# szaguldo-kamaz/FRI-ReinforcementLearning-C

Hardware: AMD Instinct MI355X
Metric: rule-distance evals/sec (rules x envs) (higher is better)
Workload: dtype f64; 1 GPU; cfg4_acrobot_64k_x_8k_per_gpu; nant=5, universe_len=41, rules_per_env=65536, envs_per_gpu=8192, exact_hits=4, dist_backend=none, world_size=1

## Files before the change

fri-reinforcementlearning-c_amd/csrc/device_common.h:

```cpp
#pragma once

#include <hip/hip_runtime.h>
#include <stdint.h>

#include "../../include/frirl_hip.h"

#define FRIRL_WAVE 64
#define FRIRL_BLOCK 256
#define FRIRL_WAVES_PER_BLOCK (FRIRL_BLOCK / FRIRL_WAVE)

namespace frirl {

__device__ __forceinline__ unsigned snap_index(const double *__restrict__ uni, int len, double point, double div)
{
    const int low = (int)((point - uni[0]) / div);
    if (low < 0) return 0u;
    if (low >= len) return (unsigned)(len - 1);
    if (low + 1 >= len) return (unsigned)low;
    const double d1 = uni[low] - point;
    const double d2 = uni[low + 1] - point;
    return (fabs(d1) <= fabs(d2)) ? (unsigned)low : (unsigned)(low + 1);
}

__device__ __forceinline__ double universe_div(const double *__restrict__ uni, int U)
// ... 95 lines not shown
namespace frirl_host {
void set_error(const char *fmt, ...);
int check_device();
int check_launch(const char *what);
int check_tables(const frirl_hip_tables *t);
int check_rulebases(const frirl_hip_tables *t, const frirl_hip_rulebases *b);
int check_demo_kind(const frirl_hip_tables *t, const frirl_hip_agent *agent, const char *who);
int check_grid_len(const frirl_hip_tables *t, const frirl_hip_agent *agent, const char *who);
int check_policy_args(const frirl_hip_tables *t, const frirl_hip_rulebases *b, const frirl_hip_agent *agent, const char *who);
int check_policy_io(const frirl_hip_agent_io *io, bool begin, const char *who);
#define FRIRL_POLICY_NANT_CASES(M) M(2) M(3) M(4) M(5) M(6) M(7) M(8)
int check_agent_shape(const frirl_hip_tables *t, const frirl_hip_rulebases *b, const frirl_hip_agent *agent, const frirl_hip_envs *envs,
                      const char *who);
inline hipStream_t as_stream(void *s) { return reinterpret_cast<hipStream_t>(s); }

struct DeviceGuard {
    int prev = -1;
    DeviceGuard() { if (hipGetDevice(&prev) != hipSuccess) { prev = -1; (void)hipGetLastError(); } }
    ~DeviceGuard() { if (prev >= 0) (void)hipSetDevice(prev); }
    DeviceGuard(const DeviceGuard &) = delete;
    DeviceGuard &operator=(const DeviceGuard &) = delete;
};

struct Options {
    int no_uidx;
    int rd_unroll;
    int rd_chunk;
    int rd_nt;
    int rd_persist;
    int rd_order;
    int rd_packed;
    int rd_sqdiff;
    int rd_qpass;
    int rd_prepass;
    int rd_coded;
    int step_wave;
    int step_track;
    int lanes_slices;
    int lanes_wpe;
    int rollout_group;
    int rollout_slices;
    int rollout_resident;
    int rollout_cap;
    int rollout_pair;
    int rollout_wps;
    int rollout_batch_resident;
    int rollout_batch_resident_rules;
    int rollout_batch_slices;
    int rollout_record_slices;
    int policy_group;
    int policy_slices;
    int learn_slices;
    int learn_alone;
    int learn_persistent;
    int multi_loopback;
    int mirror_sync;
    int no_many;
};
const Options &opts();
}
```

fri-reinforcementlearning-c_amd/csrc/learn.hip:

```cpp
#include "learn_kernel.h"

using namespace frirl_host;
int frirl_check_episode(const frirl_hip_tables *t, const frirl_hip_rulebases *b, const frirl_hip_agent *agent, const frirl_hip_envs *envs, const char *who);

static long learn_lanes()
{
    int cus = 256;
    { int dev = 0, n = 0; if (hipGetDevice(&dev) == hipSuccess && hipDeviceGetAttribute(&n, hipDeviceAttributeMultiprocessorCount, dev) == hipSuccess && n > 0) cus = n; }
    return (long)cus * 4 * 2 * FRIRL_WAVE;
}

static int learn_slices(int nlive)
{
    { const int v = opts().learn_slices; if (v == 1 || v == 2 || v == 4 || v == 8 || v == 16 || v == 32 || v == 64) return v; }
    const long lanes = learn_lanes();
    int H = 1;
    while (H < 64 && (long)nlive * (2 * H) <= lanes) H *= 2;
    return H;
}

extern "C" int frirl_hip_learn_plan(int32_t nlive, int32_t mean_rules, int32_t *slices, int32_t *agents_per_launch)
{
    if (nlive < 1 || !slices || !agents_per_launch) { set_error("frirl_hip_learn_plan: bad arguments"); return FRIRL_HIP_EINVAL; }
    const long lanes = learn_lanes();
// ... 33 lines not shown
}

static size_t learn_entries(int nlive, int maxR, int H)
{
    const int EPW = FRIRL_WAVE / H;
    const size_t tiles = ((size_t)nlive + EPW - 1) / EPW, njmax = ((size_t)maxR + H - 1) / H;
    return tiles * (njmax + frirl::LR_PADROWS) * 64;
}

extern "C" size_t frirl_hip_learn_workspace_bytes(int32_t nant, int32_t E, int32_t maxR, int32_t A)
{
    if (nant < 1 || E < 1 || maxR < 1 || A < 1) return 0;
    size_t m = 0;
    for (int H : {1, 2, 4, 8, 16, 32, 64}) { const size_t n = learn_entries(E, maxR, H); m = n > m ? n : m; }
    return m * (16 + 8 + 8) + 256;
}

#ifdef LEARN_TIMING
static unsigned long long *learn_timing_buffer()
{
    static unsigned long long *p = nullptr;
    if (!p) { if (hipMalloc(&p, 16 * 8) != hipSuccess) return nullptr; (void)hipMemset(p, 0, 16 * 8); }
    return p;
}
extern "C" int frirl_hip_learn_timing(unsigned long long *out16)
{
    unsigned long long *p = learn_timing_buffer();
    if (!p || hipMemcpy(out16, p, 16 * 8, hipMemcpyDeviceToHost) != hipSuccess) return FRIRL_HIP_EINVAL;
    (void)hipMemset(p, 0, 16 * 8);
    return FRIRL_HIP_OK;
}
#endif

extern "C" int frirl_hip_learn_run(const frirl_hip_tables *t, const frirl_hip_rulebases *b, const frirl_hip_agent *agent, const frirl_hip_envs *envs,
                                   const frirl_hip_convergence *conv, const int32_t *live, int32_t nlive, int32_t budget_steps, int32_t max_episodes,
                                   int64_t *work, int64_t *steps_total, void *workspace, size_t workspace_bytes, void *stream)
{
    int rc = frirl_check_episode(t, b, agent, envs, "frirl_hip_learn_run");
    if (rc) return rc;
    if (!conv || !conv->prev_nrules || !conv->prev_steps || !conv->prev_reward || !conv->prev_rconc || !conv->converged || !conv->episodes) { set_error("frirl_hip_learn_run: NULL convergence state"); return FRIRL_HIP_EINVAL; }
    if (!frirl_hip_learn_supported(t->nant, t->U, agent->A, agent->p, agent->env_kind)) { set_error("frirl_hip_learn_run: shape nant=%d U=%d A=%d p=%d not covered (use frirl_hip_episode_run_lanes)", t->nant, t->U, agent->A, agent->p); return FRIRL_HIP_EINVAL; }
    if (!b->uidx) { set_error("frirl_hip_learn_run: needs the 16-bit index mirror (frirl_hip_rulebases.uidx)"); return FRIRL_HIP_EINVAL; }
    if (nlive < 1 || nlive > b->E || budget_steps < 0 || max_episodes < 1) { set_error("frirl_hip_learn_run: nlive=%d / budget=%d / max_episodes=%d", nlive, budget_steps, max_episodes); return FRIRL_HIP_EINVAL; }
    if (!workspace || (reinterpret_cast<uintptr_t>(workspace) & 15)) { set_error("frirl_hip_learn_run: workspace must be a 16-byte aligned device buffer"); return FRIRL_HIP_EINVAL; }
    const size_t need = frirl_hip_learn_workspace_bytes(t->nant, nlive, b->maxR, agent->A);
    if (workspace_bytes < need) { set_error("frirl_hip_learn_run: workspace %zu B < %zu B (frirl_hip_learn_workspace_bytes)", workspace_bytes, need); return FRIRL_HIP_EINVAL; }
    hipStream_t s = as_stream(stream);
    frirl::LearnArgs la = {};
    la.u = t->u; la.ve = t->ve; la.U = t->U;
    la.Ti = static_cast<uint32_t *>(workspace);
    la.live = live; la.nlive = nlive;
    la.rb = b->rb; la.uidx = b->uidx; la.nrules = b->nrules; la.maxR = b->maxR;
    la.work = work; la.steps_total = steps_total; la.budget = budget_steps; la.max_episodes = max_episodes;
#ifdef LEARN_TIMING
    la.timing = learn_timing_buffer();
#endif
    int H = learn_slices(nlive);
    if (H < learn_min_slices(agent->A)) H = learn_min_slices(agent->A);
    if (t->nant == 3) frirl_learn_launch_mountaincar(H, t, b, agent, envs, conv, la, s);
    else if (agent->A == 3) { if (H <= 8) frirl_learn_launch_acrobot_lo(H, t, b, agent, envs, conv, la, s); else frirl_learn_launch_acrobot_hi(H, t, b, agent, envs, conv, la, s); }
    else { if (H <= 8) frirl_learn_launch_cartpole_lo(H, t, b, agent, envs, conv, la, s); else frirl_learn_launch_cartpole_hi(H, t, b, agent, envs, conv, la, s); }
    return check_launch("frirl_hip_learn_run");
}


namespace {
constexpr int LQ_BLOCK = 1024, LQ_BINS = 4096;

__global__ void learn_queue_init_kernel(int32_t *q, int n)
{
    for (int i = blockIdx.x * blockDim.x + threadIdx.x; i < n; i += gridDim.x * blockDim.x) q[i] = i;
}

__global__ __launch_bounds__(LQ_BLOCK) void learn_queue_sort_kernel(const int32_t *__restrict__ q, int take, const int32_t *__restrict__ nrules, int shift,
                                                                    int32_t *__restrict__ live)
{
    __shared__ int bins[LQ_BINS];
    __shared__ int part[LQ_BLOCK];
    for (int i = threadIdx.x; i < LQ_BINS; i += LQ_BLOCK) bins[i] = 0;
    __syncthreads();
    auto key = [&](int e) { const int k = nrules[e] >> shift; return k < 0 ? 0 : (k >= LQ_BINS ? LQ_BINS - 1 : k); };
    for (int i = threadIdx.x; i < take; i += LQ_BLOCK) atomicAdd(&bins[key(q[i])], 1);
    __syncthreads();
    constexpr int PER = LQ_BINS / LQ_BLOCK;
    int loc[PER], sum = 0;
#pragma unroll
    for (int x = 0; x < PER; x++) { loc[x] = sum; sum += bins[threadIdx.x * PER + x]; }
    part[threadIdx.x] = sum;
    __syncthreads();
    for (int off = 1; off < LQ_BLOCK; off <<= 1) {
        const int v = threadIdx.x >= off ? part[threadIdx.x - off] : 0;
        __syncthreads();
        part[threadIdx.x] += v;
        __syncthreads();
    }
    const int base = part[threadIdx.x] - sum;
#pragma unroll
    for (int x = 0; x < PER; x++) bins[threadIdx.x * PER + x] = base + loc[x];
    __syncthreads();
    for (int i = threadIdx.x; i < take; i += LQ_BLOCK) { const int e = q[i]; live[atomicAdd(&bins[key(e)], 1)] = e; }
}

__global__ __launch_bounds__(LQ_BLOCK) void learn_queue_next_kernel(const int32_t *__restrict__ q, int n, int take, const int32_t *__restrict__ live,
                                                                    const int32_t *__restrict__ converged, const int32_t *__restrict__ episodes, int max_episodes,
                                                                    const int32_t *__restrict__ nrules, const int32_t *__restrict__ status, uint8_t *refused,
                                                                    int32_t *__restrict__ nq, long long *counters)
// ... 85 lines not shown
```

fri-reinforcementlearning-c_amd/csrc/learn_kernel.h:

```cpp
#pragma once
#include "sweeps.h"
#include "envs.h"
#include <type_traits>

namespace frirl {

#ifndef LEARN_UR
#define LEARN_UR 2
#endif
constexpr int LR_BLOCK = 256;
constexpr int LR_PADROWS = 16;
constexpr int LR_WPB = LR_BLOCK / FRIRL_WAVE;
constexpr int LR_MW = 16;

struct LearnArgs {
    const double *u, *ve;
    int U;
    uint32_t *Ti;
    double *Tq;
    double *Tp;
    const int32_t *live;
    int nlive, tiles, njmax;
    double *rb;
    uint16_t *uidx;
    int32_t *nrules;
    int maxR;
    int64_t *work;
    int64_t *steps_total;
    int budget;
    long long *sum_rules;
    int max_episodes;
#ifdef LEARN_TIMING
    unsigned long long *timing;
#endif
};
#ifdef LEARN_TIMING
#define LT_MARK(i) do { const unsigned long long now_ = clock64(); if ((__ffsll((long long)__ballot(1)) - 1) == lane) { tim_s[wave][i] += now_ - tim_s[wave][15]; tim_s[wave][15] = now_; } } while (0)
#else
#define LT_MARK(i) do { } while (0)
#endif

template <int NANT, int BITS>
__global__ __launch_bounds__(256) void learn_import_kernel(const LearnArgs la, int H, const double *__restrict__ prev_rconc)
{
    constexpr int FPW = Packed<BITS>::FPW, W = Packed<BITS>::words(NANT);
    const int tile = blockIdx.x, EPW = FRIRL_WAVE / H;
    const int lane = threadIdx.x & 63, il = lane / H, h = lane % H;
    const int slot = tile * EPW + il;
    const bool exists = slot < la.nlive;
    const int e = exists ? (la.live ? la.live[slot] : slot) : 0;
    const int R = exists ? la.nrules[e] : 0;
    const int nj = (R + H - 1) / H;
    if (threadIdx.x < 64 && h == 0 && exists) atomicAdd(reinterpret_cast<unsigned long long *>(la.sum_rules), (unsigned long long)R);
    int njw = nj;
    for (int off = 32; off > 0; off >>= 1) { const int o = __shfl_xor(njw, off, FRIRL_WAVE); njw = o > njw ? o : njw; }
    for (int j = threadIdx.x / 64; j < njw; j += 4) {
        const int r = j * H + h;
        uint32_t w[W];
#pragma unroll
        for (int x = 0; x < W; x++) w[x] = 0u;
        double q = 0.0, p = 0.0;
        if (r < R) {
#pragma unroll
            for (int k = 0; k < NANT; k++) w[k / FPW] |= (uint32_t)la.uidx[((size_t)e * NANT + k) * la.maxR + r] << (BITS * (k % FPW));
            q = la.rb[((size_t)e * (NANT + 1) + NANT) * la.maxR + r];
            p = prev_rconc[(size_t)e * la.maxR + r];
        }
        const size_t o = ((size_t)tile * (la.njmax + LR_PADROWS) + LR_PADROWS + j) * 64 + lane;
#pragma unroll
        for (int x = 0; x < W; x++) la.Ti[o * W + x] = w[x];
        la.Tq[o] = q;
        la.Tp[o] = p;
    }
}

template <int NANT>
__global__ __launch_bounds__(256) void learn_export_kernel(const LearnArgs la, int H, double *__restrict__ prev_rconc)
{
    constexpr int nant = NANT;
    const int tile = blockIdx.x, EPW = FRIRL_WAVE / H;
    const int lane = threadIdx.x & 63, il = lane / H, h = lane % H;
    const int slot = tile * EPW + il;
    const bool exists = slot < la.nlive;
    const int e = exists ? (la.live ? la.live[slot] : slot) : 0;
    const int R = exists ? la.nrules[e] : 0;
    const int nj = (R + H - 1) / H;
    int njw = nj;
    for (int off = 32; off > 0; off >>= 1) { const int o = __shfl_xor(njw, off, FRIRL_WAVE); njw = o > njw ? o : njw; }
    for (int j = threadIdx.x / 64; j < njw; j += 4) {
        const int r = j * H + h;
        if (r < R) {
            const size_t o = ((size_t)tile * (la.njmax + LR_PADROWS) + LR_PADROWS + j) * 64 + lane;
            la.rb[((size_t)e * (nant + 1) + nant) * la.maxR + r] = la.Tq[o];
            prev_rconc[(size_t)e * la.maxR + r] = la.Tp[o];
        }
    }
}

template <int NANT, int NA, int KIND, int H, int BITS, int WPS>
__global__ __launch_bounds__(LR_BLOCK, WPS) void learn_kernel(const LearnArgs la, const frirl_hip_agent ag, const frirl_hip_envs ev,
                                                              const frirl_hip_convergence cv)
{
    constexpr int NS = NANT - 1, EPW = FRIRL_WAVE / H;
    constexpr int FPW = Packed<BITS>::FPW, W = Packed<BITS>::words(NANT);
    constexpr int UR = LEARN_UR;
    using RecI = typename std::conditional<W == 1, uint32_t, typename std::conditional<W == 2, uint2, uint4>::type>::type;
    static_assert(BITS == 6 || BITS == 10, "the LDS tables are laid out for 6-bit (<= 64 points) or 10-bit (<= 1024 points: cartpole) universe indices");
    constexpr int TS = 1 << BITS;
    constexpr int MW = BITS == 6 ? LR_MW : LR_MW / 2;
    constexpr bool LU = KIND != FRIRL_HIP_ENV_CARTPOLE;
    constexpr int NCOLD = 2 * NS + 2 * NANT + 3 + 4;
    __shared__ double tab_s[(LU ? 2 : 1) * NANT * TS];
    __shared__ double grid_s[NANT * FRIRL_HIP_MAX_GRID];
    __shared__ double udiv[8];
    __shared__ unsigned aidx_s[NA];
    extern __shared__ __attribute__((aligned(16))) double cold_s[];
    __shared__ uint32_t mask_s[MW * LR_BLOCK];
    static_assert(32 % (2 * UR) == 0, "a flag word is filled by whole loop iterations");
    const int U = la.U, maxR = la.maxR;
    const int lane = threadIdx.x & (FRIRL_WAVE - 1), wave = threadIdx.x / FRIRL_WAVE;
    const int il = lane / H, h = lane % H;
    const int tile = blockIdx.x * LR_WPB + wave;
    const int slot = tile * EPW + il;
    const bool exists = tile < la.tiles && slot < la.nlive;
    const int e = exists ? (la.live ? la.live[slot] : slot) : 0;
    for (int i = threadIdx.x; i < NANT * U; i += LR_BLOCK) tab_s[(i / U) * TS + i % U] = la.ve[i];
    if (LU) for (int i = threadIdx.x; i < NANT * U; i += LR_BLOCK) tab_s[NANT * TS + (i / U) * TS + i % U] = la.u[i];
    for (int i = threadIdx.x; i < NANT * FRIRL_HIP_MAX_GRID; i += LR_BLOCK) grid_s[i] = ag.grid_values[i];
    __syncthreads();
    const double *ves = tab_s, *us;
    if constexpr (LU) us = tab_s + NANT * TS; else us = la.u;
    const int USTR = LU ? TS : U;
    if ((int)threadIdx.x < NANT) udiv[threadIdx.x] = universe_div(us + (size_t)threadIdx.x * USTR, U);
    __syncthreads();
    auto locate = [&](int k, double x, unsigned &idx) { const double *uni = us + (size_t)k * USTR; idx = snap_index(uni, U, x, udiv[k]); return ves[(size_t)k * TS + idx]; };
    if ((int)threadIdx.x < NA) aidx_s[threadIdx.x] = snap_index(us + (size_t)NS * USTR, U, grid_s[NS * FRIRL_HIP_MAX_GRID + threadIdx.x], udiv[NS]);
    __syncthreads();
    auto pack = [&](uint32_t (&w)[W], int k, unsigned idx) { w[k / FPW] |= (idx & ((1u << BITS) - 1u)) << (BITS * (k % FPW)); };
    const size_t tbase = ((size_t)(tile < la.tiles ? tile : 0) * (la.njmax + LR_PADROWS) + LR_PADROWS) * 64;
    const RecI *Ti_l = reinterpret_cast<const RecI *>(la.Ti) + tbase + lane;
    double *Tq_l = la.Tq + tbase + lane, *Tp_l = la.Tp + tbase + lane;
    RecI *Ti_g = reinterpret_cast<RecI *>(la.Ti) + tbase + il * H;
    double *Tq_g = la.Tq + tbase + il * H;
    const auto pk = pin_pow(PowC<NANT>());

    auto decode = [&](const RecI &x, double (&c)[NANT]) {
        uint32_t w[W];
        if constexpr (W == 1) { w[0] = x; } else if constexpr (W == 2) { w[0] = x.x; w[1] = x.y; } else { w[0] = x.x; w[1] = x.y; w[2] = x.z; if constexpr (W > 3) w[3] = x.w; }
#pragma unroll
        for (int k = 0; k < NANT; k++) {
            constexpr uint32_t FM = ((1u << BITS) - 1u) << 3;
            const int sh = BITS * (k % FPW);
            const uint32_t off = (sh >= 3 ? (w[k / FPW] >> (sh - 3)) : (w[k / FPW] << (3 - sh))) & FM;
            c[k] = *reinterpret_cast<const double *>(reinterpret_cast<const char *>(ves + k * TS) + off);
        }
    };
    auto fetch = [&](RecI(&xi)[UR], double(&xq)[UR], int jtop, bool needq) {
        const RecI *pi = Ti_l + (long)jtop * 64;
        const double *pq = Tq_l + (long)jtop * 64;
#pragma unroll
        for (int t = 0; t < UR; t++) {
            xi[t] = pi[-t * 64];
            xq[t] = needq ? pq[-t * 64] : 0.0;
        }
    };
    struct Pref { RecI i[UR]; double q[UR]; int jt; };
    auto slice_prefetch = [&](int R, bool needq) {
        Pref p;
        p.jt = (R - h + H - 1) / H - 1;
        if (p.jt < -1) p.jt = -1;
// ... 4 lines not shown
        constexpr bool FL = decltype(flags)::value;
        RecI ib[UR];
        double qb[UR];
        uint32_t cmask = 0u;
        auto consume = [&](const RecI(&xi)[UR], const double(&xq)[UR], int jtop) {
#pragma unroll
            for (int t = 0; t < UR; t++) {
                const int j = jtop - t;
                if constexpr (FL) {
                    uint32_t hi = 0u;
                    if (j >= 0) { double c[NANT]; decode(xi[t], c); hi = f(j * H + h, c, xq[t]); }
                    cmask = __builtin_amdgcn_alignbit(cmask, hi, 31);
                } else {
                    if (j >= 0) { double c[NANT]; decode(xi[t], c); f(j * H + h, c, xq[t]); }
                }
            }
        };
        int jt = p.jt;
        const int jt0 = jt, jtm = jt & 31;
        while (jt >= 0) {
            fetch(ib, qb, jt - UR, needq);
            consume(p.i, p.q, jt);
            fetch(p.i, p.q, jt - 2 * UR, needq);
            consume(ib, qb, jt - UR);
            jt -= 2 * UR;
            if constexpr (FL) {
                if ((jt & 31) == jtm) {
                    const int wd = ((jt0 - jt) >> 5) - 1;
                    if (wd < MW) mask_s[wd * LR_BLOCK + threadIdx.x] = cmask;
                }
            }
        }
        if constexpr (FL) {
            const int done = jt0 - jt, rem = done & 31;
            if (jt0 >= 0 && rem != 0 && (done >> 5) < MW) mask_s[(done >> 5) * LR_BLOCK + threadIdx.x] = cmask << (32 - rem);
        }
    };
    auto for_slice = [&](int R, bool needq, auto &&f) {
        Pref p = slice_prefetch(R, needq);
        for_slice_from(p, needq, f, std::false_type());
    };
    auto group_or = [&](bool v) -> bool {
        const unsigned long long b = __ballot(v ? 1 : 0);
        if constexpr (H == 64) return b != 0ull;
        else return ((b >> (il * H)) & ((1ull << H) - 1ull)) != 0ull;
    };

    double states[NS], q_ant[NANT], total = 0.0, prev_reward = 0.0;
    int R = 0, fus = 0, steps = 0, prevR = 0, prev_steps = 0, nep = 0, lsteps = 0;
    bool active = false, begin = false, converged = false, refused = false;
    uint32_t episode = 0;
    long long wmain = 0, wextra = 0;
    double thr = 0.0;
    constexpr long long STEP_RULES = 24 * H;
    const long long work_budget = (long long)la.budget * (*la.sum_rules / (la.nlive > 0 ? la.nlive : 1) + STEP_RULES);
    double ve1[NANT];
    uint32_t pk1[W];
    bool ongrid = false;
#pragma unroll
    for (int k = 0; k < NS; k++) states[k] = exists ? ev.states[(size_t)e * NS + k] : 0.0;
#pragma unroll
    for (int k = 0; k < NANT; k++) q_ant[k] = exists ? ev.q_ant[(size_t)e * NANT + k] : 0.0;
#pragma unroll
    for (int x = 0; x < W; x++) pk1[x] = 0u;
#pragma unroll
    for (int k = 0; k < NANT; k++) { unsigned i1; ve1[k] = locate(k, q_ant[k], i1); pack(pk1, k, i1); }
    if (exists) {
        R = la.nrules[e]; fus = ev.fus[e]; steps = ev.ep_steps[e]; total = ev.ep_reward[e];
        begin = ev.done[e] != 0;
        episode = ev.episode ? (uint32_t)ev.episode[e] : 0u;
        prevR = cv.prev_nrules[e]; prev_steps = cv.prev_steps[e]; prev_reward = cv.prev_reward[e];
        converged = cv.converged[e] != 0; nep = cv.episodes[e];
        active = !converged && nep < la.max_episodes - 1 && la.budget > 0;
    }

#ifdef LEARN_TIMING
    __shared__ unsigned long long tim_s[LR_WPB][16];
    if (lane < 16) tim_s[wave][lane] = 0ull;
    if (lane == 0) tim_s[wave][15] = clock64();
#endif
    while (__any(active ? 1 : 0)) {
        double cur[NS], cur_q[NANT], ve2[NS], reward = 0.0;
        uint32_t pk2[W];
        int success = 0;
#pragma unroll
        for (int x = 0; x < W; x++) pk2[x] = 0u;
        Pref pmain = slice_prefetch(active ? R : 0, true);
        if (active) {
            if (begin) {
#pragma unroll
                for (int k = 0; k < NS; k++) {
                    const double v = ev.start_states ? ev.start_states[(size_t)e * NS + k] : ag.values_def[k];
                    states[k] = v; cur[k] = v; cur_q[k] = v; q_ant[k] = v;
                }
                steps = 0; total = 0.0;
            } else {
                env_do_action(KIND, q_ant[NS], states, cur);
                env_get_reward(KIND, cur, reward, success);
                env_quantize(KIND, NS, grid_s, ag.grid_len, ag.grid_div, cur, cur_q);
            }
#pragma unroll
            for (int k = 0; k < NS; k++) { unsigned i2; ve2[k] = locate(k, cur_q[k], i2); pack(pk2, k, i2); }
        } else {
#pragma unroll
            for (int k = 0; k < NS; k++) { ve2[k] = 0.0; cur[k] = 0.0; cur_q[k] = 0.0; }
        }

        LT_MARK(0);
        double *cold = cold_s + (size_t)(wave * EPW + il) * NCOLD;
        if (h == 0) {
#pragma unroll
            for (int k = 0; k < NS; k++) { cold[k] = states[k]; cold[NS + k] = cur[k]; }
#pragma unroll
            for (int k = 0; k < NANT; k++) { cold[2 * NS + k] = q_ant[k]; cold[2 * NS + NANT + k] = cur_q[k]; }
            cold[2 * NS + 2 * NANT] = total; cold[2 * NS + 2 * NANT + 1] = prev_reward; cold[2 * NS + 2 * NANT + 2] = reward;
            int *ci = reinterpret_cast<int *>(cold + 2 * NS + 2 * NANT + 3);
            ci[0] = fus; ci[1] = steps; ci[2] = prevR; ci[3] = prev_steps; ci[4] = nep; ci[5] = lsteps; ci[6] = (int)episode; ci[7] = success;
        }
        asm volatile("" ::: "memory");
        LT_MARK(1);

        double bv = 0.0, swb = 0.0;
        int ci = 0;
        unsigned hit1 = FRIRL_HIP_NO_HIT;
        double vs1 = 0.0, ws1 = 0.0;
        auto part = [&](auto a0c, auto napc, auto withpc, Pref &pf) {
            constexpr int A0 = decltype(a0c)::value, NAP = decltype(napc)::value;
            constexpr bool WITHP = decltype(withpc)::value;
            constexpr int NCP = NAP + (WITHP ? 1 : 0);
            double sv[NCP], sw[NCP], pave[NAP];
            unsigned sh[NCP];
#pragma unroll
            for (int i = 0; i < NCP; i++) { sv[i] = 0.0; sw[i] = 0.0; sh[i] = FRIRL_HIP_NO_HIT; }
#pragma unroll
            for (int a = 0; a < NAP; a++) pave[a] = ag.action_ve[A0 + a];
            if (active) {
                for_slice_from(pf, true, [&](int r, const double (&c)[NANT], double cq) {
                    const double e0 = ve2[0] - c[0];
                    double s2 = e0 * e0, s1 = 0.0;
                    if constexpr (WITHP) { const double g0 = ve1[0] - c[0]; s1 = g0 * g0; }
#pragma unroll
                    for (int k = 1; k < NS; k++) {
                        const double d2 = ve2[k] - c[k];
                        s2 = __fma_rn(d2, d2, s2);
                        if constexpr (WITHP) { const double d1 = ve1[k] - c[k]; s1 = __fma_rn(d1, d1, s1); }
                    }
                    const double va = c[NS];
#pragma unroll
                    for (int a = 0; a < NAP; a++) {
                        const double ea = pave[a] - va;
                        const double d = __fma_rn(ea, ea, s2);
                        sh[a] = (d == 0.0) ? (unsigned)r : sh[a];
                        const double wi = shepard_w(d, pk);
                        sv[a] = __fma_rn(wi, cq, sv[a]);
                        sw[a] = sw[a] + wi;
                    }
                    if constexpr (WITHP) {
                        const double e1 = ve1[NS] - va;
                        const double d = __fma_rn(e1, e1, s1);
                        sh[NAP] = (d == 0.0) ? (unsigned)r : sh[NAP];
                        const double wi = shepard_w(d, pk);
                        sv[NAP] = __fma_rn(wi, cq, sv[NAP]);
                        sw[NAP] = sw[NAP] + wi;
                        return (uint32_t)__double2hiint(thr - wi);
                    } else {
                        return 0u;
                    }
                }, std::integral_constant<bool, WITHP>());
            }
            if (H > 1) {
                constexpr int CH = 4;
#pragma unroll
                for (int i0 = 0; i0 < NCP; i0 += CH) {
                    for (int off = 1; off < H; off <<= 1) {
                        double tv[CH], tw[CH];
                        unsigned th[CH];
#pragma unroll
                        for (int i = 0; i < CH; i++) if (i0 + i < NCP) { tv[i] = __shfl_xor(sv[i0 + i], off, FRIRL_WAVE); tw[i] = __shfl_xor(sw[i0 + i], off, FRIRL_WAVE); th[i] = (unsigned)__shfl_xor((int)sh[i0 + i], off, FRIRL_WAVE); }
#pragma unroll
                        for (int i = 0; i < CH; i++) if (i0 + i < NCP) { sv[i0 + i] = sv[i0 + i] + tv[i]; sw[i0 + i] = sw[i0 + i] + tw[i]; sh[i0 + i] = th[i] < sh[i0 + i] ? th[i] : sh[i0 + i]; }
                    }
                }
            }
            if (active) {
#pragma unroll
                for (int a = 0; a < NAP; a++) {
                    const double c = (sh[a] != FRIRL_HIP_NO_HIT) ? Tq_g[(size_t)(sh[a] / H) * 64 + (sh[a] % H)] : sv[a] / sw[a];
                    if (A0 + a == 0 || bv < c) { bv = c; ci = A0 + a; swb = sw[a]; }
                }
                if constexpr (WITHP) { hit1 = sh[NAP]; vs1 = sv[NAP]; ws1 = sw[NAP]; }
            }
        };
        if constexpr (NA <= 8) {
            part(std::integral_constant<int, 0>(), std::integral_constant<int, NA>(), std::true_type(), pmain);
        } else {
            constexpr int NA1 = (NA + 1) / 2;
            part(std::integral_constant<int, 0>(), std::integral_constant<int, NA1>(), std::false_type(), pmain);
            Pref p2 = slice_prefetch(active ? R : 0, true);
            part(std::integral_constant<int, NA1>(), std::integral_constant<int, NA - NA1>(), std::true_type(), p2);
        }
        if (active) wmain += R;
        LT_MARK(2);
        auto action_conclusion = [&](int ax, double &v, double &w, unsigned &hh) {
            const double avx = ag.action_ve[ax];
            v = 0.0; w = 0.0; hh = FRIRL_HIP_NO_HIT;
            for_slice(R, true, [&](int r, const double (&c)[NANT], double cq) {
                const double e0 = ve2[0] - c[0];
                double s2 = e0 * e0;
#pragma unroll
                for (int k = 1; k < NS; k++) { const double d2 = ve2[k] - c[k]; s2 = __fma_rn(d2, d2, s2); }
                const double ea = avx - c[NS];
                const double d = __fma_rn(ea, ea, s2);
                hh = (d == 0.0) ? (unsigned)r : hh;
                const double wi = shepard_w(d, pk);
                v = __fma_rn(wi, cq, v);
                w = w + wi;
            });
            for (int off = 1; off < H; off <<= 1) {
                const double tv = __shfl_xor(v, off, FRIRL_WAVE), tw = __shfl_xor(w, off, FRIRL_WAVE);
                const unsigned th = (unsigned)__shfl_xor((int)hh, off, FRIRL_WAVE);
                v = v + tv; w = w + tw; hh = th < hh ? th : hh;
            }
            wextra += R;
        };
        asm volatile("" ::: "memory");
        {
#pragma unroll
            for (int k = 0; k < NS; k++) { states[k] = cold[k]; cur[k] = cold[NS + k]; }
#pragma unroll
            for (int k = 0; k < NANT; k++) { q_ant[k] = cold[2 * NS + k]; cur_q[k] = cold[2 * NS + NANT + k]; }
            total = cold[2 * NS + 2 * NANT]; prev_reward = cold[2 * NS + 2 * NANT + 1]; reward = cold[2 * NS + 2 * NANT + 2];
            const int *cint = reinterpret_cast<const int *>(cold + 2 * NS + 2 * NANT + 3);
            fus = cint[0]; steps = cint[1]; prevR = cint[2]; prev_steps = cint[3]; nep = cint[4]; lsteps = cint[5]; episode = (uint32_t)cint[6]; success = cint[7];
        }
        LT_MARK(3);
        if (active) {
            if (begin) {
                episode++;
                const int a0 = e_greedy(ag, ci, (uint32_t)e, episode, 0u);
                q_ant[NS] = grid_s[NS * FRIRL_HIP_MAX_GRID + a0];
                begin = false;
                double w0 = swb;
                if (a0 != ci) { double v0; unsigned h0; action_conclusion(a0, v0, w0, h0); }
                thr = (ag.weight_significant * (1.0 - 4e-9)) * w0;
#pragma unroll
                for (int k = 0; k < NS; k++) ve1[k] = ve2[k];
                ve1[NS] = ves[NS * TS + aidx_s[a0]];
#pragma unroll
                for (int x = 0; x < W; x++) pk1[x] = pk2[x];
                pack(pk1, NS, aidx_s[a0]);
                {
                    double sq[NS];
                    env_quantize(KIND, NS, grid_s, ag.grid_len, ag.grid_div, q_ant, sq);
                    ongrid = KIND != FRIRL_HIP_ENV_CARTPOLE;
#pragma unroll
                    for (int k = 0; k < NS; k++) ongrid = ongrid && (sq[k] == q_ant[k]);
                }
            } else {
                const int chosen = e_greedy(ag, ci, (uint32_t)e, episode, (uint32_t)steps + 1u);
                const bool flags_known = thr > 0.0 && thr < __builtin_inf();
                double qp = bv, w0 = swb;
                if (chosen != ci) {
                    double v;
                    unsigned hh;
                    action_conclusion(chosen, v, w0, hh);
                    qp = (hh != FRIRL_HIP_NO_HIT) ? Tq_g[(size_t)(hh / H) * 64 + (hh % H)] : v / w0;
                }
                thr = (ag.weight_significant * (1.0 - 4e-9)) * w0;
                const double qnow = (hit1 != FRIRL_HIP_NO_HIT) ? Tq_g[(size_t)(hit1 / H) * 64 + (hit1 % H)] : vs1 / ws1;
                cur_q[NS] = grid_s[NS * FRIRL_HIP_MAX_GRID + chosen];

                LT_MARK(4);
                if (!ag.evaluate) {
                    const double qdiff = ag.alpha * (reward + ag.gamma * qp - qnow);
                    bool finished = false;
                    if (qdiff > ag.qdiff_pos_boundary || qdiff < ag.qdiff_neg_boundary) {
                        double rant[NANT], ve3[NANT];
                        uint32_t pk3[W];
#pragma unroll
                        for (int k = 0; k < NANT; k++) { rant[k] = q_ant[k]; ve3[k] = ve1[k]; }
#pragma unroll
                        for (int x = 0; x < W; x++) pk3[x] = pk1[x];
                        double v3 = vs1, w3 = ws1;
                        unsigned hit3 = hit1;
                        if (!ongrid) {
                            bool same = true;
#pragma unroll
                            for (int x = 0; x < W; x++) pk3[x] = 0u;
#pragma unroll
                            for (int k = 0; k < NANT; k++) {
                                rant[k] = check_possible_states(q_ant[k], grid_s + k * FRIRL_HIP_MAX_GRID, ag.grid_len[k]);
                                unsigned i3;
                                ve3[k] = locate(k, rant[k], i3);
                                pack(pk3, k, i3);
                                same = same && (ve3[k] == ve1[k]);
                            }
                            if (!same) {
                                v3 = 0.0; w3 = 0.0; hit3 = FRIRL_HIP_NO_HIT;
                                for_slice(R, true, [&](int r, const double (&c)[NANT], double cq) {
                                    const double d0 = ve3[0] - c[0];
                                    double s = d0 * d0;
#pragma unroll
                                    for (int k = 1; k < NANT; k++) { const double d = ve3[k] - c[k]; s = __fma_rn(d, d, s); }
                                    hit3 = (s == 0.0) ? (unsigned)r : hit3;
                                    const double wi = shepard_w(s, pk);
                                    v3 = __fma_rn(wi, cq, v3);
                                    w3 = w3 + wi;
                                });
                                for (int off = 1; off < H; off <<= 1) {
                                    const double tv = __shfl_xor(v3, off, FRIRL_WAVE), tw = __shfl_xor(w3, off, FRIRL_WAVE);
                                    const unsigned th = (unsigned)__shfl_xor((int)hit3, off, FRIRL_WAVE);
                                    v3 = v3 + tv; w3 = w3 + tw; hit3 = th < hit3 ? th : hit3;
                                }
                                wextra += R;
                            }
                        }
                        if (hit3 == FRIRL_HIP_NO_HIT) {
                            if (R >= maxR) {
                                refused = true;
                            } else {
                                if (h == 0) {
                                    RecI x;
                                    if constexpr (W == 1) { x = pk3[0]; } else if constexpr (W == 2) { x.x = pk3[0]; x.y = pk3[1]; } else { x.x = pk3[0]; x.y = pk3[1]; x.z = pk3[2]; x.w = W > 3 ? pk3[W - 1] : 0u; }
                                    const size_t o = (size_t)(R / H) * 64 + (R % H);
                                    Ti_g[o] = x;
                                    Tq_g[o] = v3 / w3 + qdiff;
#pragma unroll
                                    for (int k = 0; k < NANT; k++) {
                                        la.rb[((size_t)e * (NANT + 1) + k) * maxR + R] = ve3[k];
                                        la.uidx[((size_t)e * NANT + k) * maxR + R] = (uint16_t)((pk3[k / FPW] >> (BITS * (k % FPW))) & ((1u << BITS) - 1u));
                                        if (ev.rant) ev.rant[((size_t)e * NANT + k) * maxR + R] = rant[k];
                                    }
                                }
                                R++;
                                fus = 1;
                            }
                            finished = true;
                        } else {
                            fus = 0;
                        }
                    }
                    LT_MARK(5);
                    if (!finished) {
                        const int rules = fus ? R - 1 : R;
                        if (hit1 != FRIRL_HIP_NO_HIT && (ag.skip_rules == 0 || (ag.skip_rules == 1 && (int)hit1 < rules))) {
                            if (h == 0) Tq_g[(size_t)(hit1 / H) * 64 + (hit1 % H)] = qnow + qdiff;
                        } else if (ag.skip_rules == 1 && hit1 != FRIRL_HIP_NO_HIT && (int)hit1 == rules) {
                        } else {
                            if (ag.skip_rules == 0) fus = 0;
                            const int r_skip = fus ? R - 1 : -1;
                            if (hit1 == FRIRL_HIP_NO_HIT && h == 0 && ev.spread_ant) {
#pragma unroll
                                for (int k = 0; k < NANT; k++) ev.spread_ant[(size_t)e * NANT + k] = q_ant[k];
                                if (ev.spread_R) ev.spread_R[e] = R;
                            }
                            const double iws = 1.0 / ws1;
                            auto move = [&](int r, const double (&c)[NANT]) {
                                const double d0 = ve1[0] - c[0];
                                double s = d0 * d0;
#pragma unroll
                                for (int k = 1; k < NANT; k++) { const double d = ve1[k] - c[k]; s = __fma_rn(d, d, s); }
                                const double w = shepard_w(s, pk) * iws;
                                if (w > ag.weight_significant && r != r_skip) { const double t = qdiff * w; Tq_l[(size_t)(r / H) * 64] = qnow + t; }
                            };
                            const int jt0 = (R - h + H - 1) / H - 1;
                            if (group_or(!flags_known || jt0 >= MW * 32)) {
                                for_slice(R, false, [&](int r, const double (&c)[NANT], double) { move(r, c); });
                                wextra += R;
                            } else {
                                constexpr int NCD = 8;
                                int js[NCD], nc = 0;
#pragma unroll
                                for (int i = 0; i < NCD; i++) js[i] = 0;
                                const int nw = (jt0 + 32) >> 5;
                                for (int wd = 0; wd < nw; wd++) {
                                    uint32_t m = mask_s[wd * LR_BLOCK + threadIdx.x];
                                    while (m) {
                                        const int b = __clz(m);
                                        m &= ~(0x80000000u >> b);
                                        const int j = jt0 - (wd * 32 + b);
#pragma unroll
                                        for (int i = 0; i < NCD; i++) js[i] = (nc == i) ? j : js[i];
                                        nc++;
                                    }
                                }
                                if (group_or(nc > NCD)) {
                                    for_slice(R, false, [&](int r, const double (&c)[NANT], double) { move(r, c); });
                                    wextra += R;
                                } else {
                                    RecI xs[NCD];
#pragma unroll
                                    for (int i = 0; i < NCD; i++) xs[i] = Ti_l[(long)js[i] * 64];
#pragma unroll
                                    for (int i = 0; i < NCD; i++) if (i < nc) { double c[NANT]; decode(xs[i], c); move(js[i] * H + h, c); }
                                }
                            }
                        }
                    }
                    __threadfence_block();
                    LT_MARK(6);
                }
#pragma unroll
                for (int k = 0; k < NS; k++) { states[k] = cur[k]; q_ant[k] = cur_q[k]; ve1[k] = ve2[k]; }
                q_ant[NS] = cur_q[NS];
                ve1[NS] = ves[NS * TS + aidx_s[chosen]];
#pragma unroll
                for (int x = 0; x < W; x++) pk1[x] = pk2[x];
                pack(pk1, NS, aidx_s[chosen]);
                ongrid = KIND != FRIRL_HIP_ENV_CARTPOLE;
                steps++;
                lsteps++;
                total = total + reward;
                if (success == 1 || steps >= ag.max_steps) {
                    const bool same = prevR == R && prev_steps == steps && total > ag.reward_good_above && prev_reward == total;
                    bool moved = false;
                    const int nj = (R - h + H - 1) / H;
                    constexpr int EB = 16;
                    for (int j0 = 0; j0 < nj; j0 += EB) {
                        double qn[EB];
#pragma unroll
                        for (int t = 0; t < EB; t++) qn[t] = Tq_l[(size_t)(j0 + t < nj ? j0 + t : 0) * 64];
                        if (same) {
                            double qp[EB];
#pragma unroll
                            for (int t = 0; t < EB; t++) qp[t] = Tp_l[(size_t)(j0 + t < nj ? j0 + t : 0) * 64];
#pragma unroll
                            for (int t = 0; t < EB; t++) if (j0 + t < nj && fabs(qn[t] - qp[t]) >= ag.qdiff_final_tolerance) moved = true;
                        }
#pragma unroll
                        for (int t = 0; t < EB; t++) if (j0 + t < nj) Tp_l[(size_t)(j0 + t) * 64] = qn[t];
                    }
                    moved = group_or(moved);
                    nep++;
                    if (same && !moved) converged = true;
                    prevR = R; prev_steps = steps; prev_reward = total;
                    begin = true;
                    if (converged || nep >= la.max_episodes - 1) active = false;
                }
                LT_MARK(7);
                if (wmain + (long long)lsteps * STEP_RULES >= work_budget || lsteps >= 4 * la.budget) active = false;
            }
        }
        LT_MARK(8);
    }
#ifdef LEARN_TIMING
    if (lane < 15 && la.timing) atomicAdd(&la.timing[lane], tim_s[wave][lane]);
#endif

    if (!exists || h != 0) return;
#pragma unroll
    for (int k = 0; k < NS; k++) ev.states[(size_t)e * NS + k] = states[k];
#pragma unroll
    for (int k = 0; k < NANT; k++) ev.q_ant[(size_t)e * NANT + k] = q_ant[k];
    ev.fus[e] = fus;
// ... 65 lines not shown
```

fri-reinforcementlearning-c_amd/csrc/runtime.hip:

```cpp
#include <stdarg.h>
#include <stdio.h>
#include <stdlib.h>
#include <string.h>

#include <mutex>

#include "device_common.h"

namespace frirl_host {

static thread_local char g_err[512] = "";

void set_error(const char *fmt, ...)
{
    va_list ap;
    va_start(ap, fmt);
    vsnprintf(g_err, sizeof g_err, fmt, ap);
    va_end(ap);
}

static Options g_opts;
static std::once_flag g_opts_once;
struct OptName { const char *name, *env; int Options::*field; int def; };
static const OptName k_opts[] = {
    {"no_uidx", "FRIRL_HIP_NO_UIDX", &Options::no_uidx, 0},
    {"rd_unroll", "FRIRL_HIP_RD_UNROLL", &Options::rd_unroll, 0},
    {"rd_chunk", "FRIRL_HIP_RD_CHUNK", &Options::rd_chunk, 0},
    {"rd_nt", "FRIRL_HIP_RD_NT", &Options::rd_nt, -1},
    {"rd_persist", "FRIRL_HIP_RD_PERSIST", &Options::rd_persist, -1},
    {"rd_order", "FRIRL_HIP_RD_ORDER", &Options::rd_order, 0},
    {"rd_packed", "FRIRL_HIP_RD_PACKED", &Options::rd_packed, 1},
    {"rd_sqdiff", "FRIRL_HIP_RD_SQDIFF", &Options::rd_sqdiff, 1},
    {"rd_qpass", "FRIRL_HIP_RD_QPASS", &Options::rd_qpass, 0},
    {"rd_prepass", "FRIRL_HIP_RD_PREPASS", &Options::rd_prepass, 1},
    {"rd_coded", "FRIRL_HIP_RD_CODED", &Options::rd_coded, 1},
    {"step_wave", "FRIRL_HIP_STEP_WAVE", &Options::step_wave, -1},
    {"step_track", "FRIRL_HIP_STEP_TRACK", &Options::step_track, -1},
    {"lanes_slices", "FRIRL_HIP_LANES_SLICES", &Options::lanes_slices, 0},
    {"lanes_wpe", "FRIRL_HIP_LANES_WPE", &Options::lanes_wpe, 0},
    {"rollout_group", "FRIRL_HIP_ROLLOUT_GROUP", &Options::rollout_group, 0},
    {"rollout_slices", "FRIRL_HIP_ROLLOUT_SLICES", &Options::rollout_slices, 0},
    {"rollout_resident", "FRIRL_HIP_ROLLOUT_RESIDENT", &Options::rollout_resident, -1},
    {"rollout_cap", "FRIRL_HIP_ROLLOUT_CAP", &Options::rollout_cap, 0},
    {"rollout_pair", "FRIRL_HIP_ROLLOUT_PAIR", &Options::rollout_pair, -1},
    {"rollout_wps", "FRIRL_HIP_ROLLOUT_WPS", &Options::rollout_wps, 0},
    {"rollout_batch_resident", "FRIRL_HIP_ROLLOUT_BATCH_RESIDENT", &Options::rollout_batch_resident, -1},
    {"rollout_batch_resident_rules", "FRIRL_HIP_ROLLOUT_BATCH_RESIDENT_RULES", &Options::rollout_batch_resident_rules, 0},
    {"rollout_batch_slices", "FRIRL_HIP_ROLLOUT_BATCH_SLICES", &Options::rollout_batch_slices, 0},
    {"rollout_record_slices", "FRIRL_HIP_ROLLOUT_RECORD_SLICES", &Options::rollout_record_slices, 0},
    {"policy_group", "FRIRL_HIP_POLICY_GROUP", &Options::policy_group, 0},
    {"policy_slices", "FRIRL_HIP_POLICY_SLICES", &Options::policy_slices, 0},
    {"learn_slices", "FRIRL_HIP_LEARN_SLICES", &Options::learn_slices, 0},
    {"learn_alone", "FRIRL_HIP_LEARN_ALONE", &Options::learn_alone, 0},
    {"learn_persistent", "FRIRL_HIP_LEARN_PERSISTENT", &Options::learn_persistent, -1},
    {"multi_loopback", "FRIRL_HIP_MULTI_LOOPBACK", &Options::multi_loopback, 0},
    {"no_many", "FRIRL_HIP_NO_MANY", &Options::no_many, 0},
    {"mirror_sync", "FRIRL_HIP_MIRROR_SYNC", &Options::mirror_sync, 0},
};
static void opts_init()
{
    for (const OptName &o : k_opts) {
        const char *e = getenv(o.env);
        g_opts.*(o.field) = e ? atoi(e) : o.def;
    }
}
const Options &opts()
{
    std::call_once(g_opts_once, opts_init);
    return g_opts;
}
static const OptName *find_opt(const char *name)
{
    if (name) for (const OptName &o : k_opts) if (!strcmp(o.name, name)) return &o;
    return nullptr;
}

int check_device()
{
    static thread_local int cached = 1;
    if (cached != 1) return cached;
    int n = 0;
    hipError_t e = hipGetDeviceCount(&n);
    if (e != hipSuccess || n <= 0) {
        set_error("no usable HIP device (%s): the FRIRL hot path has no CPU fallback", e == hipSuccess ? "0 devices" : hipGetErrorString(e));
        (void)hipGetLastError();
        return FRIRL_HIP_ENODEV;
    }
    int dev = 0;
    hipDeviceProp_t p;
    if (hipGetDevice(&dev) != hipSuccess || hipGetDeviceProperties(&p, dev) != hipSuccess) {
        set_error("hipGetDeviceProperties failed");
        return FRIRL_HIP_ENODEV;
    }
    if (strncmp(p.gcnArchName, "gfx950", 6) != 0) {
        set_error("device %d is %s; this library is built for gfx950 (MI355X) only", dev, p.gcnArchName);
        return FRIRL_HIP_ENODEV;
    }
    cached = FRIRL_HIP_OK;
    return cached;
}

int check_launch(const char *what)
{
    hipError_t e = hipGetLastError();
    if (e != hipSuccess) {
        set_error("%s: %s", what, hipGetErrorString(e));
// ... 70 lines not shown
```

Before: 524.3 billion evals/s.

## Carry previous-state conclusion and candidate lists across learn steps

Adds a default-on 'learn_carry' option to the learn kernel for A<=8. It keeps the next state's chosen-action conclusion (V, W, hit) up to date while rules are appended or moved, so the next step does not re-walk the rulebase to evaluate the previous state. The main walk also records significance flags from a scaled previous threshold, and the candidate list for the move step is parked in LDS. This avoids a full rule walk in the move step. It adds register and LDS pressure and more complex bookkeeping. The metric measures rule-distance evaluations, which this learn-kernel change may not touch.

Result: no change. 524.2 billion evals/s (-0.0%).

```diff
diff --git a/fri-reinforcementlearning-c_amd/csrc/device_common.h b/fri-reinforcementlearning-c_amd/csrc/device_common.h
--- a/fri-reinforcementlearning-c_amd/csrc/device_common.h
+++ b/fri-reinforcementlearning-c_amd/csrc/device_common.h
@@ -171,6 +171,7 @@
     int policy_slices;
     int learn_slices;
     int learn_alone;
+    int learn_carry;
     int learn_persistent;
     int multi_loopback;
     int mirror_sync;
diff --git a/fri-reinforcementlearning-c_amd/csrc/learn.hip b/fri-reinforcementlearning-c_amd/csrc/learn.hip
--- a/fri-reinforcementlearning-c_amd/csrc/learn.hip
+++ b/fri-reinforcementlearning-c_amd/csrc/learn.hip
@@ -109,6 +109,7 @@
     la.live = live; la.nlive = nlive;
     la.rb = b->rb; la.uidx = b->uidx; la.nrules = b->nrules; la.maxR = b->maxR;
     la.work = work; la.steps_total = steps_total; la.budget = budget_steps; la.max_episodes = max_episodes;
+    la.carry = opts().learn_carry != 0 && agent->A <= 8;
 #ifdef LEARN_TIMING
     la.timing = learn_timing_buffer();
 #endif
diff --git a/fri-reinforcementlearning-c_amd/csrc/learn_kernel.h b/fri-reinforcementlearning-c_amd/csrc/learn_kernel.h
--- a/fri-reinforcementlearning-c_amd/csrc/learn_kernel.h
+++ b/fri-reinforcementlearning-c_amd/csrc/learn_kernel.h
@@ -5,6 +5,9 @@
 
 namespace frirl {
 
+#ifndef LEARN_RHO
+#define LEARN_RHO 0.25
+#endif
 #ifndef LEARN_UR
 #define LEARN_UR 2
 #endif
@@ -12,6 +15,7 @@
 constexpr int LR_PADROWS = 16;
 constexpr int LR_WPB = LR_BLOCK / FRIRL_WAVE;
 constexpr int LR_MW = 16;
+constexpr int LR_NCD = 8;
 
 struct LearnArgs {
     const double *u, *ve;
@@ -30,6 +34,7 @@
     int budget;
     long long *sum_rules;
     int max_episodes;
+    int carry;
 #ifdef LEARN_TIMING
     unsigned long long *timing;
 #endif
@@ -116,6 +121,9 @@
     __shared__ unsigned aidx_s[NA];
     extern __shared__ __attribute__((aligned(16))) double cold_s[];
     __shared__ uint32_t mask_s[MW * LR_BLOCK];
+    constexpr bool CARRY = NA <= 8;
+    constexpr int NCD = LR_NCD, NAC = CARRY ? NA : 1;
+    __shared__ uint16_t list_s[CARRY ? NCD * LR_BLOCK : 1];
     static_assert(32 % (2 * UR) == 0, "a flag word is filled by whole loop iterations");
     const int U = la.U, maxR = la.maxR;
     const int lane = threadIdx.x & (FRIRL_WAVE - 1), wave = threadIdx.x / FRIRL_WAVE;
@@ -226,6 +234,14 @@
     uint32_t episode = 0;
     long long wmain = 0, wextra = 0;
     double thr = 0.0;
+    const double wsm = ag.weight_significant * (1.0 - 4e-9);
+    double Vc = 0.0, Wc = 0.0;
+    unsigned hc = FRIRL_HIP_NO_HIT;
+    bool cvalid = false;
+    double thrn[NAC];
+#pragma unroll
+    for (int a = 0; a < NAC; a++) thrn[a] = 0.0;
+    int nc1 = NCD + 1;
     constexpr long long STEP_RULES = 24 * H;
     const long long work_budget = (long long)la.budget * (*la.sum_rules / (la.nlive > 0 ? la.nlive : 1) + STEP_RULES);
     double ve1[NANT];
@@ -279,6 +295,21 @@
 #pragma unroll
             for (int k = 0; k < NS; k++) { ve2[k] = 0.0; cur[k] = 0.0; cur_q[k] = 0.0; }
         }
+        const bool carried = CARRY && la.carry != 0 && !__any((active && !cvalid) ? 1 : 0);
+        double thra[NAC];
+        unsigned fok = 0u;
+        if (carried) {
+            uint32_t diff = 0u;
+#pragma unroll
+            for (int k = 0; k < NS; k++) diff |= ((pk2[k / FPW] ^ pk1[k / FPW]) >> (BITS * (k % FPW))) & ((1u << BITS) - 1u);
+            const double rho = diff == 0u ? 1.0 : LEARN_RHO;
+#pragma unroll
+            for (int a = 0; a < NAC; a++) thra[a] = rho * thrn[a];
+        } else {
+#pragma unroll
+            for (int a = 0; a < NAC; a++) thra[a] = 0.0;
+            nc1 = NCD + 1;
+        }
 
         LT_MARK(0);
         double *cold = cold_s + (size_t)(wave * EPW + il) * NCOLD;
@@ -298,9 +329,12 @@
         int ci = 0;
         unsigned hit1 = FRIRL_HIP_NO_HIT;
         double vs1 = 0.0, ws1 = 0.0;
-        auto part = [&](auto a0c, auto napc, auto withpc, Pref &pf) {
-            constexpr int A0 = decltype(a0c)::value, NAP = decltype(napc)::value;
-            constexpr bool WITHP = decltype(withpc)::value;
+        double svb = 0.0;
+        unsigned shb = FRIRL_HIP_NO_HIT;
+        auto part = [&](auto a0c, auto napc, auto modec, Pref &pf) {
+            constexpr int A0 = decltype(a0c)::value, NAP = decltype(napc)::value, MODE = decltype(modec)::value;
+            constexpr bool WITHP = MODE == 1;
+            static_assert(MODE != 2 || (A0 == 0 && NAP == NAC), "flags for every action need all of them in one walk");
             constexpr int NCP = NAP + (WITHP ? 1 : 0);
             double sv[NCP], sw[NCP], pave[NAP];
             unsigned sh[NCP];
@@ -320,6 +354,7 @@
                         if constexpr (WITHP) { const double d1 = ve1[k] - c[k]; s1 = __fma_rn(d1, d1, s1); }
                     }
                     const double va = c[NS];
+                    uint32_t fl = 0u;
 #pragma unroll
                     for (int a = 0; a < NAP; a++) {
                         const double ea = pave[a] - va;
@@ -328,7 +363,9 @@
                         const double wi = shepard_w(d, pk);
                         sv[a] = __fma_rn(wi, cq, sv[a]);
                         sw[a] = sw[a] + wi;
+                        if constexpr (MODE == 2) fl |= (uint32_t)__double2hiint(thra[a] - wi);
                     }
+                    if constexpr (MODE == 2) return fl;
                     if constexpr (WITHP) {
                         const double e1 = ve1[NS] - va;
                         const double d = __fma_rn(e1, e1, s1);
@@ -340,7 +377,7 @@
                     } else {
                         return 0u;
                     }
-                }, std::integral_constant<bool, WITHP>());
+                }, std::integral_constant<bool, MODE != 0>());
             }
             if (H > 1) {
                 constexpr int CH = 4;
@@ -360,18 +397,33 @@
 #pragma unroll
                 for (int a = 0; a < NAP; a++) {
                     const double c = (sh[a] != FRIRL_HIP_NO_HIT) ? Tq_g[(size_t)(sh[a] / H) * 64 + (sh[a] % H)] : sv[a] / sw[a];
-                    if (A0 + a == 0 || bv < c) { bv = c; ci = A0 + a; swb = sw[a]; }
+                    if (A0 + a == 0 || bv < c) { bv = c; ci = A0 + a; swb = sw[a]; svb = sv[a]; shb = sh[a]; }
                 }
                 if constexpr (WITHP) { hit1 = sh[NAP]; vs1 = sv[NAP]; ws1 = sw[NAP]; }
+                if constexpr (CARRY) {
+#pragma unroll
+                    for (int a = 0; a < NAP; a++) {
+                        const double t = wsm * sw[a];
+                        if constexpr (MODE == 2) fok |= (thra[A0 + a] <= t ? 1u : 0u) << a;
+                        thrn[A0 + a] = t < __builtin_inf() ? t : thrn[A0 + a];
+                    }
+                }
             }
         };
+        using I0 = std::integral_constant<int, 0>;
+        using I1 = std::integral_constant<int, 1>;
         if constexpr (NA <= 8) {
-            part(std::integral_constant<int, 0>(), std::integral_constant<int, NA>(), std::true_type(), pmain);
+            if (carried) {
+                part(I0(), std::integral_constant<int, NA>(), std::integral_constant<int, 2>(), pmain);
+                hit1 = hc; vs1 = Vc; ws1 = Wc;
+            } else {
+                part(I0(), std::integral_constant<int, NA>(), I1(), pmain);
+            }
         } else {
             constexpr int NA1 = (NA + 1) / 2;
-            part(std::integral_constant<int, 0>(), std::integral_constant<int, NA1>(), std::false_type(), pmain);
+            part(I0(), std::integral_constant<int, NA1>(), I0(), pmain);
             Pref p2 = slice_prefetch(active ? R : 0, true);
-            part(std::integral_constant<int, NA1>(), std::integral_constant<int, NA - NA1>(), std::true_type(), p2);
+            part(std::integral_constant<int, NA1>(), std::integral_constant<int, NA - NA1>(), I1(), p2);
         }
         if (active) wmain += R;
         LT_MARK(2);
@@ -408,15 +460,39 @@
             fus = cint[0]; steps = cint[1]; prevR = cint[2]; prev_steps = cint[3]; nep = cint[4]; lsteps = cint[5]; episode = (uint32_t)cint[6]; success = cint[7];
         }
         LT_MARK(3);
+        auto park_flags = [&](bool known, int Rs, bool appended) {
+            const int jt0 = (Rs - h + H - 1) / H - 1;
+            int nc = NCD + 1;
+            if (known && hc == FRIRL_HIP_NO_HIT && jt0 < MW * 32) {
+                nc = 0;
+                const int nw = (jt0 + 32) >> 5;
+                for (int wd = 0; wd < nw; wd++) {
+                    uint32_t m = mask_s[wd * LR_BLOCK + threadIdx.x];
+                    while (m) {
+                        const int b = __clz(m);
+                        m &= ~(0x80000000u >> b);
+                        if (nc < NCD) list_s[nc * LR_BLOCK + threadIdx.x] = (uint16_t)(jt0 - (wd * 32 + b));
+                        nc++;
+                    }
+                }
+                if (appended && (R - 1) % H == h) {
+                    if (nc < NCD) list_s[nc * LR_BLOCK + threadIdx.x] = (uint16_t)((R - 1) / H);
+                    nc++;
+                }
+            }
+            nc1 = nc;
+        };
         if (active) {
             if (begin) {
                 episode++;
                 const int a0 = e_greedy(ag, ci, (uint32_t)e, episode, 0u);
                 q_ant[NS] = grid_s[NS * FRIRL_HIP_MAX_GRID + a0];
                 begin = false;
-                double w0 = swb;
-                if (a0 != ci) { double v0; unsigned h0; action_conclusion(a0, v0, w0, h0); }
-                thr = (ag.weight_significant * (1.0 - 4e-9)) * w0;
+                double w0 = swb, v0 = svb;
+                unsigned h0 = shb;
+                if (a0 != ci) action_conclusion(a0, v0, w0, h0);
+                thr = wsm * w0;
+                if constexpr (CARRY) { Vc = v0; Wc = w0; hc = h0; cvalid = true; park_flags(((fok >> a0) & 1u) != 0u, R, false); }
 #pragma unroll
                 for (int k = 0; k < NS; k++) ve1[k] = ve2[k];
                 ve1[NS] = ves[NS * TS + aidx_s[a0]];
@@ -433,14 +509,25 @@
             } else {
                 const int chosen = e_greedy(ag, ci, (uint32_t)e, episode, (uint32_t)steps + 1u);
                 const bool flags_known = thr > 0.0 && thr < __builtin_inf();
-                double qp = bv, w0 = swb;
+                double qp = bv, w0 = swb, v = svb;
+                unsigned hh = shb;
                 if (chosen != ci) {
-                    double v;
-                    unsigned hh;
                     action_conclusion(chosen, v, w0, hh);
                     qp = (hh != FRIRL_HIP_NO_HIT) ? Tq_g[(size_t)(hh / H) * 64 + (hh % H)] : v / w0;
                 }
-                thr = (ag.weight_significant * (1.0 - 4e-9)) * w0;
+                thr = wsm * w0;
+                const bool carry = CARRY && la.carry != 0;
+                const double vea = ves[NS * TS + aidx_s[chosen]];
+                if constexpr (CARRY) { Vc = v; Wc = w0; hc = hh; cvalid = true; }
+                auto d2next = [&](const double (&c)[NANT]) {
+                    const double e0 = ve2[0] - c[0];
+                    double s = e0 * e0;
+#pragma unroll
+                    for (int k = 1; k < NS; k++) { const double d = ve2[k] - c[k]; s = __fma_rn(d, d, s); }
+                    const double ea = vea - c[NS];
+                    return __fma_rn(ea, ea, s);
+                };
+                bool appended = false;
                 const double qnow = (hit1 != FRIRL_HIP_NO_HIT) ? Tq_g[(size_t)(hit1 / H) * 64 + (hit1 % H)] : vs1 / ws1;
                 cur_q[NS] = grid_s[NS * FRIRL_HIP_MAX_GRID + chosen];
 
@@ -493,12 +580,24 @@
                             if (R >= maxR) {
                                 refused = true;
                             } else {
+                                const double q3 = v3 / w3 + qdiff;
+                                if (carry) {
+                                    const double d = d2next(ve3);
+                                    if (d == 0.0) {
+                                        hc = (hc == FRIRL_HIP_NO_HIT) ? (unsigned)R : hc;
+                                    } else {
+                                        const double w = shepard_w(d, pk);
+                                        Vc = __fma_rn(w, q3, Vc);
+                                        Wc = Wc + w;
+                                    }
+                                    appended = true;
+                                }
                                 if (h == 0) {
                                     RecI x;
                                     if constexpr (W == 1) { x = pk3[0]; } else if constexpr (W == 2) { x.x = pk3[0]; x.y = pk3[1]; } else { x.x = pk3[0]; x.y = pk3[1]; x.z = pk3[2]; x.w = W > 3 ? pk3[W - 1] : 0u; }
                                     const size_t o = (size_t)(R / H) * 64 + (R % H);
                                     Ti_g[o] = x;
-                                    Tq_g[o] = v3 / w3 + qdiff;
+                                    Tq_g[o] = q3;
 #pragma unroll
                                     for (int k = 0; k < NANT; k++) {
                                         la.rb[((size_t)e * (NANT + 1) + k) * maxR + R] = ve3[k];
@@ -519,6 +618,10 @@
                         const int rules = fus ? R - 1 : R;
                         if (hit1 != FRIRL_HIP_NO_HIT && (ag.skip_rules == 0 || (ag.skip_rules == 1 && (int)hit1 < rules))) {
                             if (h == 0) Tq_g[(size_t)(hit1 / H) * 64 + (hit1 % H)] = qnow + qdiff;
+                            if (carry) {
+                                const double d = d2next(ve1);
+                                if (d != 0.0) Vc = __fma_rn(shepard_w(d, pk), (qnow + qdiff) - qnow, Vc);
+                            }
                         } else if (ag.skip_rules == 1 && hit1 != FRIRL_HIP_NO_HIT && (int)hit1 == rules) {
                         } else {
                             if (ag.skip_rules == 0) fus = 0;
@@ -529,51 +632,71 @@
                                 if (ev.spread_R) ev.spread_R[e] = R;
                             }
                             const double iws = 1.0 / ws1;
+                            double dV = 0.0;
                             auto move = [&](int r, const double (&c)[NANT]) {
                                 const double d0 = ve1[0] - c[0];
                                 double s = d0 * d0;
 #pragma unroll
                                 for (int k = 1; k < NANT; k++) { const double d = ve1[k] - c[k]; s = __fma_rn(d, d, s); }
                                 const double w = shepard_w(s, pk) * iws;
-                                if (w > ag.weight_significant && r != r_skip) { const double t = qdiff * w; Tq_l[(size_t)(r / H) * 64] = qnow + t; }
+                                if (w > ag.weight_significant && r != r_skip) {
+                                    const double t = qdiff * w, qn = qnow + t;
+                                    double *q = Tq_l + (size_t)(r / H) * 64;
+                                    if (carry) {
+                                        const double dn = d2next(c);
+                                        if (dn != 0.0) dV = __fma_rn(shepard_w(dn, pk), qn - *q, dV);
+                                    }
+                                    *q = qn;
+                                }
                             };
-                            const int jt0 = (R - h + H - 1) / H - 1;
-                            if (group_or(!flags_known || jt0 >= MW * 32)) {
+                            int js[NCD], nc = 0;
+#pragma unroll
+                            for (int i = 0; i < NCD; i++) js[i] = 0;
+                            if (carried) {
+                                if constexpr (CARRY) {
+                                    nc = nc1;
+#pragma unroll
+                                    for (int i = 0; i < NCD; i++) js[i] = i < nc ? (int)list_s[i * LR_BLOCK + threadIdx.x] : 0;
+                                }
+                            } else {
+                                const int jt0 = (R - h + H - 1) / H - 1;
+                                if (!flags_known || jt0 >= MW * 32) {
+                                    nc = NCD + 1;
+                                } else {
+                                    const int nw = (jt0 + 32) >> 5;
+                                    for (int wd = 0; wd < nw; wd++) {
+                                        uint32_t m = mask_s[wd * LR_BLOCK + threadIdx.x];
+                                        while (m) {
+                                            const int b = __clz(m);
+                                            m &= ~(0x80000000u >> b);
+                                            const int j = jt0 - (wd * 32 + b);
+#pragma unroll
+                                            for (int i = 0; i < NCD; i++) js[i] = (nc == i) ? j : js[i];
+                                            nc++;
+                                        }
+                                    }
+                                }
+                            }
+                            if (group_or(nc > NCD)) {
                                 for_slice(R, false, [&](int r, const double (&c)[NANT], double) { move(r, c); });
                                 wextra += R;
                             } else {
-                                constexpr int NCD = 8;
-                                int js[NCD], nc = 0;
-#pragma unroll
-                                for (int i = 0; i < NCD; i++) js[i] = 0;
-                                const int nw = (jt0 + 32) >> 5;
-                                for (int wd = 0; wd < nw; wd++) {
-                                    uint32_t m = mask_s[wd * LR_BLOCK + threadIdx.x];
-                                    while (m) {
-                                        const int b = __clz(m);
-                                        m &= ~(0x80000000u >> b);
-                                        const int j = jt0 - (wd * 32 + b);
-#pragma unroll
-                                        for (int i = 0; i < NCD; i++) js[i] = (nc == i) ? j : js[i];
-                                        nc++;
-                                    }
-                                }
-                                if (group_or(nc > NCD)) {
-                                    for_slice(R, false, [&](int r, const double (&c)[NANT], double) { move(r, c); });
-                                    wextra += R;
-                                } else {
-                                    RecI xs[NCD];
-#pragma unroll
-                                    for (int i = 0; i < NCD; i++) xs[i] = Ti_l[(long)js[i] * 64];
-#pragma unroll
-                                    for (int i = 0; i < NCD; i++) if (i < nc) { double c[NANT]; decode(xs[i], c); move(js[i] * H + h, c); }
-                                }
+                                RecI xs[NCD];
+#pragma unroll
+                                for (int i = 0; i < NCD; i++) xs[i] = Ti_l[(long)js[i] * 64];
+#pragma unroll
+                                for (int i = 0; i < NCD; i++) if (i < nc) { double c[NANT]; decode(xs[i], c); move(js[i] * H + h, c); }
+                            }
+                            if (carry) {
+                                for (int off = 1; off < H; off <<= 1) dV = dV + __shfl_xor(dV, off, FRIRL_WAVE);
+                                Vc = Vc + dV;
                             }
                         }
                     }
                     __threadfence_block();
                     LT_MARK(6);
                 }
+                if constexpr (CARRY) { if (carry) park_flags(((fok >> chosen) & 1u) != 0u, appended ? R - 1 : R, appended); }
 #pragma unroll
                 for (int k = 0; k < NS; k++) { states[k] = cur[k]; q_ant[k] = cur_q[k]; ve1[k] = ve2[k]; }
                 q_ant[NS] = cur_q[NS];
diff --git a/fri-reinforcementlearning-c_amd/csrc/runtime.hip b/fri-reinforcementlearning-c_amd/csrc/runtime.hip
--- a/fri-reinforcementlearning-c_amd/csrc/runtime.hip
+++ b/fri-reinforcementlearning-c_amd/csrc/runtime.hip
@@ -52,6 +52,7 @@
     {"policy_slices", "FRIRL_HIP_POLICY_SLICES", &Options::policy_slices, 0},
     {"learn_slices", "FRIRL_HIP_LEARN_SLICES", &Options::learn_slices, 0},
     {"learn_alone", "FRIRL_HIP_LEARN_ALONE", &Options::learn_alone, 0},
+    {"learn_carry", "FRIRL_HIP_LEARN_CARRY", &Options::learn_carry, 1},
     {"learn_persistent", "FRIRL_HIP_LEARN_PERSISTENT", &Options::learn_persistent, -1},
     {"multi_loopback", "FRIRL_HIP_MULTI_LOOPBACK", &Options::multi_loopback, 0},
     {"no_many", "FRIRL_HIP_NO_MANY", &Options::no_many, 0},
```
